# AlgoLab/RecGraph

Measured on AMD Instinct MI355X. Metric: aligned reads/sec (-m 8 recombination, 1 kbp reads, 10k-row/32-path graph), higher is better.
Workload: dtype int16

## Files before the change

### recgraph_amd/csrc/rg_path_driver.hip

```cpp
#include <algorithm>
#include <chrono>
#include <cstdio>
#include <cstdlib>
#include <cstring>

#include "gap/rg_path_gap.hpp"
#include "gap_local/rg_path_gap_local.hpp"
#include "gap_long/rg_path_gap_long.hpp"
#include "gap_xlong/rg_path_gap_xlong.hpp"
#include "gap_xstrands/rg_gap_xstrands.hpp"
#include "edit/rg_path_edit.hpp"
#include "edit_xlong/rg_path_edit_xlong.hpp"
#include "edit_strands/rg_edit_strands.hpp"
#include "rg_kernel_timer.hpp"
#include "rg_path_kernels.hpp"
#include "rg_path_plan.hpp"

namespace rg {

struct PathWorkImpl {
    bool tables = false;
    DevBuf<int> fpoff, fprow, fpslot, rpoff, rprow, rpslot;
    DevBuf<ReadState> state;
    DevBuf<int> roll, mf, wr, mfarg, wrarg, thr, flayer, rlayer;
// ... 433 lines not shown
    RG_TRY(T.run("k_search", [&] { return launch_search(sr, chunk, stream); }));
    RG_TRY(T.inst(launch_need(w.state.p, w.nf.p, w.nr.p, plan.use_rec ? w.nrec.p : nullptr, plan.use_rec ? w.nrrec.p : nullptr, w.need.p, chunk, stream)));
    if (plan.spec) RG_TRY(T.inst(launch_verify(w.state.p, w.lb.p, w.need.p + 4, w.rt_flags.p, chunk, sa.dsel_pick, sa.dsel_pick2, sa.dsel_lo, sa.dsel_hi, stream)));
    return RG_OK;
}

int Run::enqueue_tail() {
    const int C = plan.C;
    LayerArgs la;
    memset(&la, 0, sizeof la);
    la.semi = plan.semi ? 1 : 0;
    la.nwv = plan.nwv;
    la.g = gd; la.sc = sc; la.reads = d_reads; la.read_off = off(); la.state = w.state.p; la.dir_words = plan.dir_words; la.dir_fmt = plan.use16 ? 1 : 0;
    la.layer_stride = plan.layer_stride; la.fpoff = w.fpoff.p; la.fprow = w.fprow.p; la.fpslot = w.fpslot.p;
    la.rpoff = w.rpoff.p; la.rprow = w.rprow.p; la.rpslot = w.rpslot.p;
    la.rev = 0; la.dirs = w.fdirs.p; la.dirs_stride = plan.fdirs_stride; la.layer = w.flayer.p;
    const int win = plan.layer_window;
    auto layer = [&]() {
        if (win) return launch_layer_window(la, chunk, C, win, stream);
        return plan.layer16 ? launch_layer16(la, chunk, C, stream) : launch_layer(la, chunk, C, stream);
    };
    auto fwd_side = [&]() { la.rev = 0; la.dirs = w.fdirs.p; la.dirs_stride = plan.fdirs_stride; la.layer = w.flayer.p; };
    auto rev_side = [&]() { la.rev = 1; la.dirs = w.rdirs.p; la.dirs_stride = plan.rdirs_stride; la.layer = w.rlayer.p; };
    const char* family = win ? LAYER_WINDOW_LOG : "inst:";
    RG_TRY(T.run("k_layer_fwd", layer, family, win != 0));
    if (plan.mode == RG_MODE_RECOMBINATION) {
        rev_side();
        RG_TRY(T.run("k_layer_rev", layer, family, win != 0));
    }
    TraceArgs ta;
    memset(&ta, 0, sizeof ta);
    ta.g = gd; ta.sc = sc; ta.reads = d_reads; ta.read_off = off(); ta.state = w.state.p; ta.rec = d_rec + done;
    ta.ops = d_ops + (long long)done * ops_stride; ta.ops_stride = ops_stride; ta.flayer = w.flayer.p;
    ta.rlayer = w.rlayer.p; ta.layer_stride = plan.layer_stride; ta.fpoff = w.fpoff.p; ta.fprow = w.fprow.p;
    ta.rpoff = w.rpoff.p; ta.rprow = w.rprow.p; ta.nreads = chunk; ta.mode = p.mode; ta.semi = plan.semi ? 1 : 0; ta.nwv = plan.nwv;
    ta.window = win; ta.nfull = w.need.p + NEED_LAYER_FULL;
    RG_TRY(T.run("k_trace", [&] { return launch_trace(ta, C, stream); }));
    if (win) {
        la.only_full = 1;
        fwd_side();
        RG_TRY(T.run("k_layer_full", [&] { return launch_layer16(la, chunk, C, stream); }));
        if (plan.mode == RG_MODE_RECOMBINATION) {
            rev_side();
            RG_TRY(T.run("k_layer_full", [&] { return launch_layer16(la, chunk, C, stream); }));
        }
        ta.window = 0; ta.only_full = 1;
        RG_TRY(T.run("k_trace_full", [&] { return launch_trace(ta, C, stream); }));
    }
    return read_back();
}

int Run::read_back() {
    HIPCHK(hipMemcpyAsync(w.h_sum, d_cells, sizeof(unsigned long long), hipMemcpyDeviceToHost, stream));
    HIPCHK(hipMemcpyAsync(w.h_sum + 5, d_cells + 1, sizeof(unsigned long long), hipMemcpyDeviceToHost, stream));
    HIPCHK(hipMemcpyAsync(w.h_sum + 1, w.need.p, 8 * sizeof(unsigned), hipMemcpyDeviceToHost, stream));
    return T.collect(stats);
}

int Run::enqueue_chunk() {
    HIPCHK(hipMemsetAsync(w.state.p, 0, sizeof(ReadState) * chunk, stream));
    if (plan.gap) return enqueue_pathwise_gap();
    if (plan.edit_strands) return enqueue_pathwise_edit_strands();
    if (plan.edit) return plan.edit_xlong ? enqueue_pathwise_edit_xlong() : enqueue_pathwise_edit();
    SweepArgs sa = sweep_args();
    SeedArgs se;
    se.g = gd; se.state = w.state.p; se.nreads = chunk; se.mode = p.mode; se.sc = sc; se.reads = d_reads; se.read_off = off();
    int rc = plan.mode == RG_MODE_PATHWISE ? enqueue_pathwise(sa, se) : enqueue_recombination(sa, se);
    if (rc) return rc;
    return enqueue_tail();
}

int Run::dump_list_stats() {
    const unsigned* nd = need();
    std::vector<unsigned> hn(chunk), hr(chunk);
    HIPCHK(hipMemcpy(hn.data(), w.nf.p, sizeof(unsigned) * chunk, hipMemcpyDeviceToHost));
    HIPCHK(hipMemcpy(hr.data(), w.nr.p, sizeof(unsigned) * chunk, hipMemcpyDeviceToHost));
    unsigned long long sf = 0, sr = 0;
    for (int i = 0; i < chunk; ++i) { sf += hn[i]; sr += hr[i]; }
    fprintf(stderr, "[rg] chunk %d reads: fwd cand mean %.1f max %u (cap %u), rev cand mean %.1f max %u (cap %u)\n", chunk,
            (double)sf / chunk, nd[0], w.fcap, (double)sr / chunk, nd[1], w.rcap);
    if (plan.use_rec) {
        HIPCHK(hipMemcpy(hn.data(), w.nrec.p, sizeof(unsigned) * chunk, hipMemcpyDeviceToHost));
        HIPCHK(hipMemcpy(hr.data(), w.nrrec.p, sizeof(unsigned) * chunk, hipMemcpyDeviceToHost));
        sf = sr = 0;
        for (int i = 0; i < chunk; ++i) { sf += hn[i]; sr += hr[i]; }
        fprintf(stderr, "[rg] records: forward mean %.1f max %u (cap %u), reverse mean %.1f max %u (cap %u)\n",
                (double)sf / chunk, nd[2], w.frec_cap, (double)sr / chunk, nd[3], w.rrec_cap);
    }
    return RG_OK;
}

int Run::regrow_lists(bool& redo) {
    redo = false;
    if (plan.mode != RG_MODE_RECOMBINATION) return RG_OK;
    const unsigned needf = need()[0], needr = need()[1], needrec = need()[2], needrrec = need()[3];
    if (debug) {
        const int rc = dump_list_stats();
        if (rc) return rc;
    }
    if (plan.use_rec && (needrrec > w.rrec_cap || needrec > w.frec_cap)) {
        const unsigned long long fullrec = (unsigned long long)h.L * WAVE;
        if ((needrrec > w.rrec_cap && w.rrec_cap >= fullrec) || (needrec > w.frec_cap && w.frec_cap >= fullrec))
            return fail(RG_ERR_CAPACITY, "record list overflow at full size");
        while (w.rrec_cap < needrrec) w.rrec_cap = (unsigned)std::min<unsigned long long>(2ull * w.rrec_cap, fullrec);
        while (w.frec_cap < needrec) w.frec_cap = (unsigned)std::min<unsigned long long>(2ull * w.frec_cap, fullrec);
        redo = true;
    }
    if (needf > w.fcap || needr > w.rcap) {
// ... 52 lines not shown
    std::vector<uint8_t> fl((size_t)chunk);
    std::vector<long long> ho((size_t)chunk + 1);
    HIPCHK(hipMemcpy(fl.data(), w.rt_flags.p, (size_t)chunk, hipMemcpyDeviceToHost));
    HIPCHK(hipMemcpy(ho.data(), off(), sizeof(long long) * ((size_t)chunk + 1), hipMemcpyDeviceToHost));
    std::vector<int> idx;
    std::vector<long long> so(1, 0);
    for (int i = 0; i < chunk; ++i)
        if (fl[(size_t)i]) { idx.push_back(i); so.push_back(so.back() + (ho[(size_t)i + 1] - ho[(size_t)i])); }
    const int nr = (int)idx.size();
    int rc;
    if ((rc = w.rt_idx.upload(idx)) || (rc = w.rt_off.upload(so)) || (rc = w.rt_reads.alloc((size_t)so.back() + 1)) ||
        (rc = w.rt_bad.alloc((size_t)nr)) || (rc = w.rt_rec.alloc((size_t)nr)) || (rc = w.rt_ops.alloc((size_t)nr * (size_t)ops_stride)) ||
        (rc = w.rt_cells.alloc(2)))
        return rc;
    HIPCHK(hipMemsetAsync(w.rt_bad.p, 0, (size_t)nr, stream));
    RG_TRY(T.inst(launch_gather_reads(d_reads, off(), w.rt_idx.p, w.rt_off.p, w.rt_reads.p, nr, stream)));
    const PathCtx again{h, gd, p, w.retry, stream, w.rt_cells.p, 0, T, stats, spec_level + 1};
    const PathJob failed{w.rt_reads.p, w.rt_off.p, w.rt_bad.p, nr, max_n, w.rt_rec.p, w.rt_ops.p, ops_stride};
    unsigned long long c2[2] = {0, 0};
    RG_TRY(path_driver_run(again, failed, c2));
    RG_TRY(T.inst(launch_scatter_results(w.rt_idx.p, w.rt_rec.p, w.rt_ops.p, d_rec + done, d_ops + (long long)done * ops_stride, ops_stride, nr, stream)));
    HIPCHK(hipStreamSynchronize(stream));
    cells_perf += c2[1];
    return T.collect(stats);
}

}

int path_driver_vote_table(const HostGraph& h, PathWork& pw, const uint32_t** keys, unsigned* table_mask) {
    if (!pw.impl) pw.impl = new PathWorkImpl();
    const int rc = ensure_tables(h, *pw.impl);
    if (rc) return rc;
    *keys = pw.impl->kmer_keys.p;
    *table_mask = pw.impl->kmer_mask;
    return RG_OK;
}

int path_driver_run(const PathCtx& c, const PathJob& j, unsigned long long* cells ) {
    const HostGraph& h = c.h;
    const rg_params& p = c.p;
    hipStream_t stream = c.stream;
    unsigned long long* d_cells = c.d_cells;
    KernelStats& stats = c.stats;
    const int nreads = j.nreads;
    if (!c.w.impl) c.w.impl = new PathWorkImpl();
    PathWorkImpl& w = *c.w.impl;
    const Options& opt = options();
    PathPlan plan;
    int rc = plan_pathwise(p, PathPlanInput{h.P, h.L, h.fslots, h.rslots, h.max_path_rows, j.max_n}, opt, c.spec_level, plan);
    if (rc || (rc = plan_gap_stage(plan, j.stage))) return rc;
    Run r{h, c.gd, p, w, plan, j.reads, j.off, j.bad, j.max_n, j.rec, j.ops, j.ops_stride, d_cells, stream, stats, c.spec_level, c.T, opt.debug != 0};
    for (int i = 0; i < 36; ++i) r.sc.t[i] = p.scores[i];
    r.h_off = j.h_off;
    if (!w.h_sum) HIPCHK(hipHostMalloc((void**)&w.h_sum, 8 * sizeof(unsigned long long), hipHostMallocDefault));
    if ((rc = w.need.alloc(8)) || (rc = ensure_tables(h, w))) return rc;
    if (w.fcap == 0) { w.fcap = plan.fcap; w.rcap = plan.rcap; w.frec_cap = plan.frec_cap; w.rrec_cap = plan.rrec_cap; }
    size_t budget = (size_t)96 << 30;
    {
        size_t fr = 0, tot = 0;
        if (hipMemGetInfo(&fr, &tot) == hipSuccess) budget = fr / 4 * 3;
        if (c.mem_budget) budget = c.mem_budget;
    }
    unsigned long long cells_done = 0, cells_perf = 0;
    int oom_shift = 0;
    while (r.done < nreads) {
        HIPCHK(hipMemsetAsync(d_cells, 0, 2 * sizeof(unsigned long long), stream));
        HIPCHK(hipMemsetAsync(w.need.p, 0, 8 * sizeof(unsigned), stream));
        const size_t per_read_all = plan.per_read_all(w.fcap, w.rcap, w.frec_cap, w.rrec_cap);
        int maxchunk = (int)std::min<size_t>(8192, std::max<size_t>(1, (budget >> oom_shift) / per_read_all));
        if (opt.chunk_reads > 0) maxchunk = std::min<int>(maxchunk, opt.chunk_reads);
        const double dbg_t0 = r.debug ? now_s() : 0;
        const int chunk = r.chunk = (int)even_chunks(nreads - r.done, maxchunk);
        bool oom = false;
        if ((rc = r.alloc_chunk(&oom))) {
            if (rc == RG_ERR_HIP && oom && chunk > 1 && oom_shift < 12) { ++oom_shift; continue; }
            return rc;
        }
        if (r.debug) fprintf(stderr, "[rg] chunk of %d reads: buffers ready after %.1f ms\n", chunk, (now_s() - dbg_t0) * 1e3);
        if ((rc = r.enqueue_chunk())) return rc;
        if (r.debug) fprintf(stderr, "[rg] chunk of %d reads: done after %.1f ms\n", chunk, (now_s() - dbg_t0) * 1e3);
        if (r.async_err != hipSuccess) return fail(RG_ERR_HIP, std::string("hipMemsetAsync: ") + hipGetErrorString(r.async_err));
        bool redo = false;
        if ((rc = r.regrow_lists(redo))) return rc;
        if (redo) continue;
        const unsigned long long chunk_cells = w.h_sum[0];
        cells_perf += w.h_sum[5];
        const unsigned nretry = r.nretry();
        if (r.debug && (plan.spec || plan.spec4)) fprintf(stderr, "[rg] speculative bound (margin %d): %u of %d reads did not reach it\n", plan.spec_margin, nretry, chunk);
        if (r.debug && plan.spec4 && nretry && (rc = r.dump_spec4_retries())) return rc;
        if (r.debug && plan.dsel && (rc = r.dump_dsel_retries())) return rc;
        if (plan.layer_window) {
            add_stat(stats, "mem:layer_full_reads", (double)r.need()[NEED_LAYER_FULL], 1);
            if (r.debug) fprintf(stderr, "[rg] layer window of %d columns: %u of %d reads took the full-width layers\n", plan.layer_window, r.need()[NEED_LAYER_FULL], chunk);
        }
        if (plan.use_rec) {
            add_stat(stats, "mem:silent_rows", (double)r.need()[NEED_SILENT_ROWS], 1);
            add_stat(stats, "mem:run_rows", (double)r.need()[NEED_RUN_ROWS], 1);
        }
        if (nretry && (rc = r.second_pass(cells_perf))) return rc;
        cells_done += chunk_cells;
        r.done += chunk;
        add_stat(stats, "mem:work_bytes_per_read", (double)per_read_all, 1);
    }
    cells[0] += cells_done;
    cells[1] += cells_perf;
    return RG_OK;
}

}
```

### recgraph_amd/csrc/rg_path_kernels.hpp

```cpp
#pragma once
#include "rg_path_args.hpp"
#include "rg_path_plan.hpp"
#include "rg_launch_log.hpp"
#include "layer_window/rg_layer_window.hpp"

namespace rg {

template <int H>
__device__ __forceinline__ void dir16_decode(unsigned w, unsigned& u16, unsigned& l16) {
    constexpr unsigned LOWH = (1u << H) - 1u;
    const unsigned t = __brev(w);
    u16 = ((t >> 24) & LOWH) | (((t >> 16) & LOWH) << H);
    l16 = ((t >> 8) & LOWH) | ((t & LOWH) << H);
}

struct SweepArgs {
    PathGraphDev g;
    DevScores sc;
    const uint8_t* reads;
    const long long* read_off;
    const uint8_t* bad;
    ReadState* state;
    int* roll;
    int rev;
    int track_best;
    const int* thr;
    const int4* fsteps;
    const int4* rsteps;
    int nfsteps, nrsteps;
    const int4* fsplit;
    const int4* rsplit;
    int use_split;
    const int* lb;
    int brc, maxmatch;
    int semi;
    float rbw;
    int* colmax_out;
    int* colarg_out;
    Cand* cand;
    unsigned cand_cap;
    unsigned* ncand_out;
    uint32_t* dirs;
    long long dirs_stride;
    int dir_words;
    unsigned long long* cells;
    int count_cells;
    int oob;
    int* frec;
    unsigned frec_cap;
    int nwv;
    int gather_ok;
    const unsigned long long* flead;
    const unsigned long long* rlead;
    const unsigned long long* fslead;
    const unsigned long long* rslead;
    int retire;
    int retire_shift;
    const int* order;
    unsigned long long table_members;
    unsigned long long fmembers, rmembers;
    const int* dsel_pick;
    const int* dsel_pick2;
    int dsel_lo, dsel_hi;
    unsigned* runstat;
};
constexpr int NEED_SILENT_ROWS = 6;
constexpr int NEED_RUN_ROWS = 7;

struct ExpandArgs {
    ReadState* state;
    const int* frec;
    unsigned frec_cap;
    const unsigned* nrec;
    Cand* fcand;
    unsigned fcap;
    unsigned* nf;
    const int* wr;
    int wpad;
    int brc;
    const int* knm;
    int rev;
    const long long* read_off;
    float rbw;
    int gcost;
};

struct SeedArgs {
    PathGraphDev g;
    ReadState* state;
    int nreads;
    int mode;
    DevScores sc;
    const uint8_t* reads;
    const long long* read_off;
};

struct ThrArgs {
    const ReadState* state;
    const int* colmax;
    int* thr;
    int wpad;
    int brc;
    int use_bound;
    const int* lb;
};

struct BoundArgs {
    PathGraphDev g;
    ReadState* state;
    const long long* read_off;
    const int* mf; const int* mfarg;
    const int* wr; const int* wrarg;
    int wpad;
    int brc;
    float mrc;
    float rbw;
};

struct Opt0Args {
    PathGraphDev g;
// ... 176 lines not shown
```

### recgraph_amd/csrc/rg_sweep16.hip

```cpp
#include <algorithm>
#include <type_traits>

#include "rg_path_kernels.hpp"
#include "rg_pk16.hpp"

namespace rg {

namespace {

constexpr int NEG32 = INT32_MIN / 4;
typedef unsigned u32x4 __attribute__((ext_vector_type(4)));
typedef unsigned u32x2 __attribute__((ext_vector_type(2)));
__device__ __forceinline__ __amdgpu_buffer_rsrc_t uniform_rsrc(const void* base, unsigned bytes) {
    const unsigned long long u = (unsigned long long)base;
    const unsigned lo = (unsigned)__builtin_amdgcn_readfirstlane((int)(unsigned)u), hi = (unsigned)__builtin_amdgcn_readfirstlane((int)(unsigned)(u >> 32));
    void* p = (void*)(((unsigned long long)hi << 32) | lo);
    return __builtin_amdgcn_make_buffer_rsrc(p, 0, (int)__builtin_amdgcn_readfirstlane((int)bytes), 0x00020000);
}

template <int C>
struct RowOps16 {
    static constexpr int H = C / 2;
    static constexpr unsigned FULL = H >= 16 ? 0xffffffffu : ((((1u << H) - 1u) << 16) | ((1u << H) - 1u));

// ... 145 lines not shown
#define RG_STALL_BEGIN() ((void)0)
#define RG_STALL_END(acc) ((void)0)
#endif

struct PathWords {
    unsigned long long w0, w1, w2, w3;
    __device__ __forceinline__ unsigned long long get(int i) const { return i == 0 ? w0 : (i == 1 ? w1 : (i == 2 ? w2 : w3)); }
    __device__ __forceinline__ void set(int i, unsigned long long v) { if (i == 0) w0 = v; else if (i == 1) w1 = v; else if (i == 2) w2 = v; else w3 = v; }
};

template <int C, int kColmax, bool kRec, bool kWide, bool kSemi>
__global__ __launch_bounds__(64, SWEEP16_WAVES) void k_sweep16(SweepArgs a) {
    static_assert(kColmax == 0 || kColmax == 1, "column maxima with their rows, or none");
    static_assert(!(kColmax == 1 && kRec), "a record sweep tracks no column maxima (k_colmax_rec reads them out of the records): launch_sweep16");
    constexpr int H = C / 2;
    constexpr bool kTrack = kColmax == 1 || kRec;
    constexpr bool kRet = ((kRec && kColmax == 0) || !kTrack) && !kSemi;
    constexpr int NW = kWide ? RG_PW : 1;
    constexpr bool kChain = !kTrack;
    constexpr int KRUN = sweep16_krun(C, !kTrack, kRec && kColmax == 0, kWide);
    static_assert(!(kRec && C <= 16) || KRUN == RG_SWEEP16_RUN_PATHS, "the split step tables (rg_steps.cpp) are built for register runs of RG_SWEEP16_RUN_PATHS paths");
    const int rd = a.order ? a.order[blockIdx.x] : blockIdx.x;
#ifdef RG_SWEEP16_STALLSTAT
    const unsigned long long st_t0 = __builtin_amdgcn_s_memtime();
    unsigned long long st_run = 0, st_nrun = 0, st_gen = 0;
#endif
    const int lane = threadIdx.x;
    const PathGraphDev& g = a.g;
    const int P = g.P;
    const int wpad = C * WAVE;
    const int wrow = H * WAVE;
    ReadState* rs = a.state + rd;
    const long long ro = a.read_off[rd];
    const int n = __builtin_amdgcn_readfirstlane((int)(a.read_off[rd + 1] - ro));
    if (a.bad[rd] || n + 1 > wpad) {
        if (lane == 0 && !a.rev) { rs->status = a.bad[rd] ? ST_BAD_BASE : ST_WOULD_PANIC; }
        return;
    }
    const uint8_t* read = a.reads + ro - 1;
    const bool rev = a.rev;
    const int ncols = rev ? n : n + 1;
    const int GAP = 5;
    extern __shared__ __attribute__((aligned(16))) int lds16[];
    constexpr int EP = kWide ? RG_MAXP : 64;
    constexpr int GTW = C * WAVE > 5 * 64 ? C * WAVE : 5 * 64;
    int* sct = lds16;
    int* endv = lds16 + 64;
    int* endr = endv + EP;
    int* gT = endr + EP;
    int* s2 = gT;
    int* sprof = gT + GTW;
    const int PR_RVL = P, PR_NPROF = P + 1;
    if (lane < 36) sct[lane] = a.sc.t[lane];
    else if (lane < 44) sct[lane] = 0;
    __syncthreads();
    const int gcost = __builtin_amdgcn_readfirstlane(sct[GAP]);
    pair_table(s2, sct, gcost, lane);
    int* rows = a.roll + (long long)rd * (P + 2) * wrow;
    const unsigned lane_row_off = (unsigned)lane * (unsigned)(H * sizeof(int));
    const __amdgpu_buffer_rsrc_t rows_rsrc = uniform_rsrc(rows, (unsigned)((P + 2) * wrow) * 4u);
    auto ld_row = [&](int k, int (&dst)[H]) {
        const int so = k * (int)(wrow * sizeof(int));
        if constexpr (H >= 4) {
#pragma unroll
            for (int r4 = 0; r4 < H / 4; ++r4) {
                const u32x4 v = __builtin_amdgcn_raw_buffer_load_b128(rows_rsrc, (int)lane_row_off + 16 * r4, so, 0);
                dst[4 * r4] = (int)v.x; dst[4 * r4 + 1] = (int)v.y; dst[4 * r4 + 2] = (int)v.z; dst[4 * r4 + 3] = (int)v.w;
            }
        } else {
            const u32x2 v = __builtin_amdgcn_raw_buffer_load_b64(rows_rsrc, (int)lane_row_off, so, 0);
            dst[0] = (int)v.x; dst[1] = (int)v.y;
        }
    };
    auto st_row = [&](int k, const int (&src)[H]) {
        const int so = k * (int)(wrow * sizeof(int));
        if constexpr (H >= 4) {
#pragma unroll
            for (int r4 = 0; r4 < H / 4; ++r4) {
                const u32x4 v = {(unsigned)src[4 * r4], (unsigned)src[4 * r4 + 1], (unsigned)src[4 * r4 + 2], (unsigned)src[4 * r4 + 3]};
                __builtin_amdgcn_raw_buffer_store_b128(v, rows_rsrc, (int)lane_row_off + 16 * r4, so, 0);
                asm volatile("s_nop 1" :: "v"(v));
            }
        } else {
            const u32x2 v = {(unsigned)src[0], (unsigned)src[1]};
            __builtin_amdgcn_raw_buffer_store_b64(v, rows_rsrc, (int)lane_row_off, so, 0);
        }
    };
    unsigned long long pcode[(H + 7) / 8] = {};
    int thrk[(kRec || !kTrack) ? 1 : C];
#define THRK(q) thrk[(kRec || !kTrack) ? 0 : (q)]
    int thz[kRec ? H : 1];
    int minplain2 = 0;
    int thzmin = 0;
    int next_eval = INT32_MAX;
    int minthrk = INT32_MAX;
    int minplain = INT32_MAX;
    const bool tight = a.thr != nullptr || a.oob;
    const int oob = max((int)((float)(n + 1) * (1.0f - a.rbw) / 2.0f), 1);
    auto thr_key = [&](int q, bool member_rule) -> int {
        const int c = lane * C + q;
        const int j = rev ? n - c : c;
        int th = INT32_MAX;
        if (c < ncols && j >= oob && j < n + 1 - oob) {
            if (a.thr) th = a.thr[(long long)rd * wpad + j];
            else if (a.lb) th = a.lb[rd] + a.brc - (n - j) * a.maxmatch;
        }
        if (th == INT32_MAX) return INT32_MAX;
// ... 297 lines not shown
    auto set_keys = [&](int (&bkey)[C], const int (&row)[H], int ks) {
        int k = ks;
        asm volatile("" : "+v"(k));
#pragma unroll
        for (int r = 0; r < H; ++r) {
            bkey[r] = (int)(((unsigned)row[r] << 16) | (unsigned)k);
            bkey[r + H] = (int)(((unsigned)row[r] & 0xffff0000u) | (unsigned)k);
        }
    };
    auto fold_keys = [&](int (&bkey)[C], const int (&row)[H], int ks) {
        int k = ks;
        asm volatile("" : "+v"(k));
#pragma unroll
        for (int r = 0; r < H; ++r) {
            bkey[r] = max(bkey[r], (int)(((unsigned)row[r] << 16) | (unsigned)k));
            bkey[r + H] = max(bkey[r + H], (int)(((unsigned)row[r] & 0xffff0000u) | (unsigned)k));
        }
    };

    auto load_steps = [&](int li_, int (&s)[H]) {
        if (li_ >= 4) [[unlikely]] {
            ld_row(PR_NPROF, s);
            __builtin_amdgcn_s_waitcnt(0x0F70);
            asm volatile("" ::: "memory");
            return;
        }
        const int* sp = sprof + (li_ * WAVE + lane) * H;
        if constexpr (H >= 4) {
#pragma unroll
            for (int r4 = 0; r4 < H / 4; ++r4) {
                const int4 v = reinterpret_cast<const int4*>(sp)[r4];
                s[4 * r4] = v.x; s[4 * r4 + 1] = v.y; s[4 * r4 + 2] = v.z; s[4 * r4 + 3] = v.w;
            }
        } else {
            const int2 v = *reinterpret_cast<const int2*>(sp);
            s[0] = v.x; s[1] = v.y;
        }
    };
    auto keys_ld = [&](int (&key)[C]) {
#pragma unroll
        for (int q = 0; q < C; ++q) key[q] = gT[q * WAVE + lane];
    };
    auto keys_st = [&](const int (&key)[C]) {
#pragma unroll
        for (int q = 0; q < C; ++q) gT[q * WAVE + lane] = key[q];
    };
    int MUw[kWide ? H : 1], MLw[kWide ? H : 1];
    unsigned lmaskw = 0;
    int srcw = 0;
    bool row_open = false;
    constexpr bool kSilent = kRec && kColmax == 0 && !kWide && !kSemi && C <= 16;
    const bool silent_ok = kSilent && (rev || (a.thr == nullptr && a.brc >= 0));
    int* sil = sct + 40;
#ifdef RG_SWEEP16_RETSTAT
    unsigned long long stat_e = 0, stat_n = 0, stat_h = 0;
#endif
    auto retire_eval = [&](int e) {
        PathWords hop{0ull, 0ull, 0ull, 0ull};
        constexpr int EB = !kTrack ? 1 : (C <= 16 ? 4 : 2);
        int rvc[H];
        ld_row(PR_RVL, rvc);
#pragma unroll
        for (int pg = 0; pg < NW; ++pg) {
            unsigned long long todo = needed.get(pg), hp = 0ull;
            while (todo) {
                int kq[EB];
                int tmp[EB][H];
#pragma unroll
                for (int u = 0; u < EB; ++u) {
                    kq[u] = -1;
                    if (todo) {
                        kq[u] = __builtin_ctzll(todo);
                        todo &= todo - 1;
                        ld_row(pg * 64 + kq[u], tmp[u]);
                    }
                }
#pragma unroll
                for (int u = 0; u < EB; ++u) {
                    if (kq[u] < 0) break;
                    int m = pk_add_sat(tmp[u][0], rvc[0]);
#pragma unroll
                    for (int r = 1; r < H; ++r) m = pk_max(m, pk_add_sat(tmp[u][r], rvc[r]));
                    const int v = max(lo16(m), hi16(m));
                    if (__builtin_amdgcn_readlane(dpp_incl_max(v, INT32_MIN), WAVE - 1) < 0) hp |= 1ull << kq[u];
                }
            }
            hop.set(pg, hp);
        }
        if constexpr (kSilent) {
            if (silent_ok) { sil[0] |= (int)(unsigned)hop.w0; sil[1] |= (int)(unsigned)(hop.w0 >> 32); }
        }
        const int nw = kWide ? (P + 63) >> 6 : 1;
        const unsigned long long* lead = (rev ? a.rlead : a.flead) + (long long)e * (64 * nw) * nw;
        PathWords nd{0ull, 0ull, 0ull, 0ull};
#pragma unroll
        for (int pg = 0; pg < NW; ++pg) nd.set(pg, needed.get(pg) & ~hop.get(pg));
#ifdef RG_SWEEP16_RETSTAT
        const unsigned long long nd_first = nd.w0;
#endif
        if constexpr (!kWide) {
            const unsigned long long lead_k = lane < P ? lead[lane] : 0ull;
            for (;;) {
                const unsigned long long ad = __ballot(((needed.w0 >> lane) & 1ull) && !((nd.w0 >> lane) & 1ull) && (lead_k & nd.w0) != 0ull);
                if (!ad) break;
                nd.w0 |= ad;
            }
// ... 2 lines not shown
                bool grown = false;
#pragma unroll
                for (int pg = 0; pg < NW; ++pg) {
                    bool leads = false;
                    if (pg < nw && pg * 64 + lane < P && ((needed.get(pg) >> lane) & 1ull) && !((nd.get(pg) >> lane) & 1ull)) {
#pragma unroll
                        for (int w = 0; w < NW; ++w)
                            if (w < nw) leads = leads || (lead[(long long)(pg * 64 + lane) * nw + w] & nd.get(w)) != 0ull;
                    }
                    const unsigned long long ad = __ballot(leads);
                    if (ad) { nd.set(pg, nd.get(pg) | ad); grown = true; }
                }
                if (!grown) break;
            }
        }
        needed = nd;
#ifdef RG_SWEEP16_RETSTAT
        stat_e += 1ull; stat_n += (unsigned long long)__popcll(nd.w0); stat_h += (unsigned long long)__popcll(nd_first);
#endif
    };
    while (t < nsteps) {
        int w0, w1;
        unsigned long long gmask;
        if (kRet && next_eval != INT32_MAX) {
            if ((t >> 6) != blk) fetch(t, w0, w1, gmask);
            if (t >= next_eval) [[unlikely]] {
                retire_eval(t >> a.retire_shift);
                next_eval = (t | ((1 << a.retire_shift) - 1)) + 1;
                live = block_live();
            }
            const unsigned long long m = live >> (t & (WAVE - 1));
            if (m == 0ull) { t = (t | (WAVE - 1)) + 1; continue; }
            t += __builtin_ctzll(m);
        }
        fetch(t, w0, w1, gmask);
        const int i = w0 & 0xfffff;
        const int li = (w0 >> 20) & 7;
        const int flags = (((w0 >> 23) & 7) == F_INNER && ((w0 >> 26) & 63) != 0) ? 7 : ((w0 >> 23) & 7);
        const int slot = w1 & 0xfffff;
        const int kbase = kWide ? ((w1 >> 29) & 3) * 64 : 0;
        const bool cont = kWide && w1 < 0;
        const int ga = kbase + ((flags & F_INNER) ? __builtin_ctzll(gmask | (1ull << 63)) : ((w0 >> 26) & 63));
        const int nm = __popcll(gmask);
        const int run_left = (flags & F_INNER) ? ((w0 >> 26) & 63) : 0;
        const int page = kWide ? (w1 >> 29) & 3 : 0;
        const unsigned long long gm = kRet ? (gmask & word_of(needed, page)) : gmask;
        const int nme = kRet ? __popcll(gm) : nm;
        if (kRet && gm == 0ull) {
            if (run_left == 0) {
                if (flags & F_FIRST) row_open = false;
                if (track && (flags & F_LAST) && row_open) {
                    int key[C];
                    keys_ld(key);
                    row_end(i, ((w1 >> 20) & 511) - 1, key);
                }
                if (flags & F_LAST) row_open = false;
            }
            ++t;
            continue;
        }
        int went = 1, wide_n = 0, wide_total = nm, wide_needed = 0;
        PathWords wide_gw{0ull, 0ull, 0ull, 0ull};
        int wide_ids[KRUN > 0 ? KRUN : 1];
        bool wide_sel = false;
        if (kWide && (flags & F_INNER) && run_left > 0) {
#pragma unroll
            for (int kk = 0; kk < KRUN; ++kk) wide_ids[kk] = 0;
            auto add = [&](unsigned long long m, int base) {
                while (m) {
                    const int id = base + __builtin_ctzll(m);
                    m &= m - 1;
#pragma unroll
                    for (int kk = 0; kk < KRUN; ++kk) if (kk == wide_n) wide_ids[kk] = id;
                    ++wide_n;
                }
            };
            add(gm, kbase);
            wide_gw.set(page, gm);
            wide_needed = nme;
            wide_sel = (gmask & word_of(dsel_w, page)) != 0ull;
            while (t + went < nsteps) {
                const int nw1 = peek_w1(t + went);
                if (nw1 >= 0) break;
                const unsigned long long mm = peek_gm(t + went);
                const int pg = (nw1 >> 29) & 3;
                wide_total += __popcll(mm);
                add(mm & word_of(needed, pg), pg * 64);
                wide_gw.set(pg, mm & word_of(needed, pg));
                wide_needed += __popcll(mm & word_of(needed, pg));
                wide_sel = wide_sel || (mm & word_of(dsel_w, pg)) != 0ull;
                ++went;
            }
        }
        const bool wide_run = kWide && KRUN > 0 && (flags & F_INNER) && run_left > 0 && wide_n >= 1 && wide_n <= KRUN;
        struct MemberIter {
            PathWords w;
            int pg;
            __device__ __forceinline__ int next() {
                while (pg < NW) {
                    const unsigned long long m = w.get(pg);
                    if (m) { w.set(pg, m & (m - 1)); return pg * 64 + __builtin_ctzll(m); }
                    ++pg;
                }
                return -1;
            }
        };
        const int g_nm = kWide ? wide_total : nm, g_nme = kWide ? wide_needed : nme;
        if ((kRec ? kColmax == 0 : !track) && a.gather_ok && !semi_end && (flags & F_INNER) && g_nm > KRUN &&
            (!kWide || run_left > 0) && (!kRet || g_nme > KRUN) && run_left * (GATHER_PER_MEMBER_ROW * (g_nm - 1) - GATHER_PER_ROW) >= GATHER_PER_MEMBER_RUN * (g_nm - 1)) {
            const int R = (w0 >> 26) & 63;
            const int ka = ga;
            int A[H], G[H];
            __syncthreads();
#pragma unroll
            for (int r = 0; r < H; ++r) A[r] = 0;
            ld_row(ka, A);
#if defined(RG_SWEEP16_STALLSTAT) && RG_SWEEP16_STALLSTAT == 2
            { RG_STALL_BEGIN(); RG_STALL_END(st_run); ++st_nrun; }
#endif
            if (kRec && track) {
                int bd[H], bk[H];
#pragma unroll
                for (int r = 0; r < H; ++r) { bd[r] = 0; bk[r] = pack16(ka, ka); }
                MemberIter it{kWide ? wide_gw : PathWords{gm, 0ull, 0ull, 0ull}, 0};
                it.w.set(ka >> 6, it.w.get(ka >> 6) & ~(1ull << (ka & 63)));
                int nx[H];
                int kn = it.next();
                if (kn >= 0) ld_row(kn, nx);
                while (kn >= 0) {
                    const int k = kn;
                    int cur[H];
#pragma unroll
                    for (int r = 0; r < H; ++r) cur[r] = nx[r];
                    kn = it.next();
                    if (kn >= 0) ld_row(kn, nx);
                    int kk = k;
                    asm volatile("" : "+v"(kk));
                    const int K2 = (int)(((unsigned)kk << 16) | (unsigned)kk);
#pragma unroll
                    for (int r = 0; r < H; ++r) {
                        const int d = pk_sub_sat(cur[r], A[r]);
                        const int lt = pk_sign(pk_sub_sat(d, bd[r]));
                        bd[r] = pk_max(bd[r], d);
                        bk[r] = bfi(lt, bk[r], K2);
                    }
                }
#pragma unroll
                for (int r = 0; r < H; ++r) {
                    gT[r * WAVE + lane] = (int)(((unsigned)bd[r] << 16) | ((unsigned)bk[r] & 0xffffu));
                    gT[(r + H) * WAVE + lane] = (int)(((unsigned)bd[r] & 0xffff0000u) | ((unsigned)bk[r] >> 16));
                }
            }
            {
                int gl = lane;
                asm volatile("" : "+v"(gl));
#pragma unroll
                for (int r = 0; r < H; ++r) { const int w = r * WAVE + gl; G[r] = pack16(2 * w, 2 * w + 1); }
            }
            __syncthreads();
            int ri = i, rli = li, rslot = slot, rw1 = w1;
            for (int step = 0;; ++step) {
                const int g_i = gcost;
                const int g0 = kSemi ? 0 : g_i;
                int s[H], MU[H], ML[H], XU[H], XL[H];
                load_steps(rli, s);
                int lmax_unused;
                RowOps16<C>::alpha(A, s, g_i, g0, lane, XU, XL, lmax_unused);
                const bool gdirs = kWide ? ((kColmax == 0 || dirs != nullptr) && (wide_sel || edge_row(ri))) : want_dirs(gmask, 0, ri);
                if (gdirs) store_dirs(rslot, XU, XL);
                const unsigned lmask = RowOps16<C>::masks(XU, XL, MU, ML);
                const int src = RowOps16<C>::src_lane(lmask, lane);
                RowOps16<C>::template member<true>(G, MU, lane, MU, ML, lmask, src);
                cells += (unsigned long long)g_nm;
                done += 2ull;
                if (kRec && track) {
                    int bv[H], K2[H];
                    constexpr int HS = 31 - __builtin_clz(H * WAVE);
// ... 114 lines not shown
            };
            constexpr bool kRowsInBody = !kChain && !kWide;
            if constexpr (!kRowsInBody) ld_run(rnm);
#if defined(RG_SWEEP16_STALLSTAT) && RG_SWEEP16_STALLSTAT == 3
            const unsigned long long st_rb = __builtin_amdgcn_s_memtime();
#endif
            int ri = i, rli = li, rslot = slot, rw1 = w1, rfl = 7;
            int rleft = run_left;
            bool tail = false;
            for (;;) {
            tail = false; rfl = 7;
            auto run_rows = [&](auto rn_tag, auto lean_tag) __attribute__((always_inline)) {
            constexpr int RN = decltype(rn_tag)::value;
            constexpr bool kLean = decltype(lean_tag)::value;
            const unsigned long long run_sel = kWide ? (wide_sel ? ~0ull : 0ull) : rgm;
            const int run_page = 0;
            if constexpr (kRowsInBody) ld_run(RN);
            unsigned nrows = 0;
            while (true) {
                int cnt = 1;
                if constexpr (!kWide) {
                    if (!tail) cnt = max(min(min(rleft, WAVE - (t & (WAVE - 1))), nsteps - t), 1);
                }
                nrows += (unsigned)cnt;
                int idx = t & (WAVE - 1);
                for (int left = cnt;;) {
                const int g_i = gcost;
                const int g0 = kSemi ? 0 : g_i;
                int XU[H], XL[H];
#if defined(RG_SWEEP16_STALLSTAT) && RG_SWEEP16_STALLSTAT == 3
                ++st_nrun;
#endif
                int s[H];
                load_steps(rli, s);
                int lmax;
                RowOps16<C>::alpha(rr[0], s, g_i, g0, lane, XU, XL, lmax);
                if constexpr (!kLean) {
                    if (kWide ? ((kColmax == 0 || dirs != nullptr) && (wide_sel || edge_row(ri))) : want_dirs(run_sel, run_page, ri)) store_dirs(rslot, XU, XL);
                }
                if constexpr (RN > 1) {
                    int MU[H], ML[H];
                    const unsigned lmask = RowOps16<C>::masks(XU, XL, MU, ML);
                    const int src = RowOps16<C>::src_lane(lmask, lane);
                    int SEL[H];
                    RowOps16<C>::select_steps(SEL, s, MU, g_i, g0, lane);
                    int zl[KRUN > 0 ? KRUN : 1], vlo[KRUN > 0 ? KRUN : 1];
#pragma unroll
                    for (int kk = 1; kk < KRUN; ++kk)
                        if (kk < RN) { RowOps16<C>::member_p1(rr[kk], SEL, MU, ML, lmask, zl[kk], vlo[kk]); zl[kk] = __shfl(zl[kk], src, WAVE); }
#pragma unroll
                    for (int kk = 1; kk < KRUN; ++kk)
                        if (kk < RN) RowOps16<C>::member_p2(rr[kk], ML, lmask, zl[kk], vlo[kk]);
                }
                if (kRec && kColmax == 0 && tail) {
                    if (track) {
                        if (rfl & F_FIRST) row_open = false;
                        int key[C];
                        if (row_open) { keys_ld(key); fold_keys(key, rr[0], mk[0]); } else set_keys(key, rr[0], mk[0]);
#pragma unroll
                        for (int kk = 1; kk < KRUN; ++kk) if (kk < RN) fold_keys(key, rr[kk], mk[kk]);
                        row_open = true;
                        int tri = ri, tw1 = rw1;
                        if constexpr (kLean) asm volatile("" : "+s"(tri), "+s"(tw1));
                        if (rfl & F_LAST) { row_end(tri, ((tw1 >> 20) & 511) - 1, key); row_open = false; }
                        else keys_st(key);
                    }
                } else if constexpr (kLean) {
                } else if (track && kRec && kColmax == 0) {
                    int bv[H];
#pragma unroll
                    for (int r = 0; r < H; ++r) bv[r] = rr[0][r];
#pragma unroll
                    for (int kk = 1; kk < KRUN; ++kk)
                        if (kk < RN) {
#pragma unroll
                            for (int r = 0; r < H; ++r) bv[r] = pk_max(bv[r], rr[kk][r]);
                        }
                    const int knm_row = ((rw1 >> 20) & 511) - 1;
                    int acc = -1;
                    bool fine = true;
                    if constexpr (RN == 1 && kRec) {
                        if (knm_row >= 0) fine = __any(((unsigned)pk_sub_sat(lmax, thzmin) & 0x80008000u) != 0x80008000u);
                    }
                    if (!fine) {
                    } else if (knm_row >= 0) [[likely]] {
#pragma unroll
                        for (int r = 0; r < H; ++r) acc &= pk_sub_sat(bv[r], thz[kRec ? r : 0]);
                    } else {
                        int m = bv[0];
#pragma unroll
                        for (int r = 1; r < H; ++r) m = pk_max(m, bv[r]);
                        acc = pk_sub_sat(m, minplain2);
                    }
                    const bool lhit = ((unsigned)acc & 0x80008000u) != 0x80008000u;
                    if (__any(lhit)) {
                        bool mine;
                        int4* rp = rec_slot(ri, lhit, mine);
#pragma unroll
                        for (int half = 0; half < 2; ++half) {
                            int hk[H];
#pragma unroll
                            for (int kk = 0; kk < KRUN; ++kk)
                                if (kk < RN) {
                                    int kv = mk[kk];
                                    asm volatile("" : "+v"(kv));
#pragma unroll
                                    for (int r = 0; r < H; ++r) {
                                        const int key = half == 0 ? (int)(((unsigned)rr[kk][r] << 16) | (unsigned)kv)
                                                                  : (int)(((unsigned)rr[kk][r] & 0xffff0000u) | (unsigned)kv);
                                        hk[r] = kk == 0 ? key : max(hk[r], key);
                                    }
                                }
                            rec_half(rp, mine, half, hk);
                        }
                    }
                } else if (track) {
                    int key[C];
                    set_keys(key, rr[0], mk[0]);
// ... 124 lines not shown
        } else {
        const int g_i = gcost;
        const int g0 = kSemi ? 0 : g_i;
        int s[H];
        load_steps(li, s);
        int MUl[kWide ? 1 : H], MLl[kWide ? 1 : H];
        unsigned lmaskl = 0;
        int srcl = 0;
        int (&MU)[H] = *reinterpret_cast<int (*)[H]>(kWide ? MUw : MUl);
        int (&ML)[H] = *reinterpret_cast<int (*)[H]>(kWide ? MLw : MLl);
        unsigned& lmask = kWide ? lmaskw : lmaskl;
        int& src = kWide ? srcw : srcl;
        {
            unsigned long long rest = cont ? gm : gm & ~(1ull << (ga - kbase));
            cells += (unsigned long long)nm;
            done += (unsigned long long)nme;
            int nxt[H];
            int knext = -1;
            if (rest) {
                knext = kbase + __builtin_ctzll(rest);
                rest &= rest - 1;
                ld_row(knext, nxt);
            }
            int key[C];
            bool have = false;
            if (track) {
                if (flags & F_FIRST) row_open = false;
                have = row_open;
                if (have) keys_ld(key);
            }
            if (!cont) {
                int rowa[H];
                ld_row(ga, rowa);
#if defined(RG_SWEEP16_STALLSTAT) && RG_SWEEP16_STALLSTAT == 1
                { RG_STALL_BEGIN(); RG_STALL_END(st_gen); }
#endif
                int XU[H], XL[H];
                int lmax_unused;
                RowOps16<C>::alpha(rowa, s, g_i, g0, lane, XU, XL, lmax_unused);
                st_row(ga, rowa);
                bool wd = want_dirs(gmask, page, i);
                if (kWide && !wd && t + 1 < nsteps) wd = peek_w1(t + 1) < 0;
                if (wd) store_dirs(slot, XU, XL);
                lmask = RowOps16<C>::masks(XU, XL, MU, ML);
                src = RowOps16<C>::src_lane(lmask, lane);
                if (track) {
                    if (!have) set_keys(key, rowa, ga); else fold_keys(key, rowa, ga);
                    have = true;
                }
                if (semi_end) end_fold(ga, i, rowa);
            }
            int SEL[H];
            RowOps16<C>::select_steps(SEL, s, MU, g_i, g0, lane);
            while (knext >= 0) {
                const int k = knext;
                int cur[H];
#pragma unroll
                for (int r = 0; r < H; ++r) cur[r] = nxt[r];
                if (rest) {
                    knext = kbase + __builtin_ctzll(rest);
                    rest &= rest - 1;
                    ld_row(knext, nxt);
                } else knext = -1;
                RowOps16<C>::member(cur, SEL, lane, MU, ML, lmask, src);
                st_row(k, cur);
                if (track) fold_keys(key, cur, k);
                if (semi_end) end_fold(k, i, cur);
            }
            if (track) {
                row_open = true;
                if (e_flags & F_LAST) row_end(e_i, ((e_w1 >> 20) & 511) - 1, key);
                else keys_st(key);
            }
        }
        }
        if (semi_end && (e_flags & F_LAST)) end_row_done(e_i);
        if (e_flags & F_LAST) row_open = false;
        if (e_adv) ++t;
    }

    if (kColmax == 1 && a.colmax_out) {
#pragma unroll
        for (int q = 0; q < C; ++q) {
            const int c = lane * C + q;
            if (c < ncols) {
                a.colmax_out[(long long)rd * wpad + (rev ? n - c : c)] = ckey[kColmax == 1 ? q : 0] == INT32_MIN ? NEG32 : (ckey[kColmax == 1 ? q : 0] >> 16) + c * gcost;
                if (a.colarg_out) a.colarg_out[(long long)rd * wpad + (rev ? n - c : c)] = (crow[kColmax == 1 ? q : 0] << 8) | (ckey[kColmax == 1 ? q : 0] & 255);
            }
        }
    }
    if (a.ncand_out && lane == 0) a.ncand_out[rd] = ncand;
    __syncthreads();
    if (!rev && !kSemi) {
        const int ql = n % C, ln = n / C;
        for (int k = lane; k < P; k += WAVE) {
            const int pv = rows[(long long)k * wrow + ln * H + (ql % H)];
            rs->sink_val[k] = (kRet && !((word_of(needed, k >> 6) >> (k & 63)) & 1ull)) ? NEG32 : (ql >= H ? hi16(pv) : lo16(pv)) + n * gcost;
        }
    }
    if (semi_end) {
        for (int k = lane; k < P; k += WAVE) { rs->sink_val[k] = endv[k]; rs->path_end_row[k] = endr[k]; }
        if (lane == ln_end) { rs->s0 = gbest_val; rs->end_row_best = gbest_row; rs->seed_path = gbest_path; }
    }
    if constexpr (kSilent) {
        if (lane == 0 && a.runstat) { atomicAdd(a.runstat, (unsigned)sil[2]); atomicAdd(a.runstat + 1, (unsigned)sil[3]); }
    }
    if (lane == 0 && a.count_cells) {
        const unsigned long long all = kRet && a.table_members ? a.table_members : cells;
#ifdef RG_SWEEP16_STALLSTAT
        {
            const unsigned long long tot = __builtin_amdgcn_s_memtime() - st_t0;
            atomicAdd(a.cells, (tot >> 8) | ((st_gen >> 8) << 32));
            atomicAdd(a.cells + 1, (st_run >> 8) | (st_nrun << 32));
            return;
        }
#endif
#ifdef RG_SWEEP16_RETSTAT
        if (kRet) { atomicAdd(a.cells, stat_e | (stat_n << 32)); atomicAdd(a.cells + 1, stat_h | ((unsigned long long)(rev ? 0 : 1) << 48)); return; }
#endif
        atomicAdd(a.cells, all * (unsigned long long)(n + 1));
        atomicAdd(a.cells + 1, done * (unsigned long long)(n + 1));
    }
}

template <int C>
__global__ __launch_bounds__(256) void k_expand(ExpandArgs a) {
    const int rd = blockIdx.x;
    const int lane = threadIdx.x & (WAVE - 1), wv = threadIdx.x / WAVE, nwv = blockDim.x / WAVE;
    ReadState* rs = a.state + rd;
    if (rs->status & (ST_BAD_BASE | ST_WOULD_PANIC)) return;
    const unsigned nrec = a.nrec[rd];
    if (nrec > a.frec_cap) { if (threadIdx.x == 0) rs->status |= ST_OVERFLOW; return; }
    const int bound = rs->bound;
    const int nread = (int)(a.read_off[rd + 1] - a.read_off[rd]);
    const int oob = max((int)((float)(nread + 1) * (1.0f - a.rbw) / 2.0f), 1);
    const int* base = a.frec + (long long)rd * a.frec_cap * (4 + C);
    Cand* out = a.fcand + (long long)rd * a.fcap;
    const int* wr = a.wr + (long long)rd * a.wpad;
    constexpr int LPR = C / 4, RPW = WAVE / LPR;
    const int part = lane % LPR, sub = lane / LPR;
    for (unsigned t0 = wv * RPW; t0 < nrec; t0 += nwv * RPW) {
        const unsigned t = t0 + sub;
        if (t >= nrec) continue;
        const int* rp = base + (long long)t * (4 + C);
        const int rl = rp[0];
        const int4 k4 = *reinterpret_cast<const int4*>(rp + 4 + 4 * part);
        const int keys[4] = {k4.x, k4.y, k4.z, k4.w};
        const int knm = a.knm[rl >> 6];
#pragma unroll
        for (int e = 0; e < 4; ++e) {
            const int cc = (rl & 63) * C + 4 * part + e;
            if (cc >= (a.rev ? nread : nread + 1)) continue;
            const int key = keys[e] + cc * a.gcost * 65536;
            const int val = key >> 16;
            const int col = a.rev ? nread - cc : cc;
            if (col < oob || col >= nread + 1 - oob) continue;
            if (val + wr[col] - a.brc < bound) continue;
            if (knm >= 0 && key <= knm) continue;
// ... 301 lines not shown
```

Baseline: 151,200.

## Skip key folds for silent paths in recombination sweep and add fold stats

```diff
diff --git a/recgraph_amd/csrc/rg_path_driver.hip b/recgraph_amd/csrc/rg_path_driver.hip
--- a/recgraph_amd/csrc/rg_path_driver.hip
+++ b/recgraph_amd/csrc/rg_path_driver.hip
@@ -509,8 +509,8 @@
 
 int Run::read_back() {
     HIPCHK(hipMemcpyAsync(w.h_sum, d_cells, sizeof(unsigned long long), hipMemcpyDeviceToHost, stream));
-    HIPCHK(hipMemcpyAsync(w.h_sum + 5, d_cells + 1, sizeof(unsigned long long), hipMemcpyDeviceToHost, stream));
-    HIPCHK(hipMemcpyAsync(w.h_sum + 1, w.need.p, 8 * sizeof(unsigned), hipMemcpyDeviceToHost, stream));
+    HIPCHK(hipMemcpyAsync(w.h_sum + 1 + NEED_WORDS / 2, d_cells + 1, sizeof(unsigned long long), hipMemcpyDeviceToHost, stream));
+    HIPCHK(hipMemcpyAsync(w.h_sum + 1, w.need.p, NEED_WORDS * sizeof(unsigned), hipMemcpyDeviceToHost, stream));
     return T.collect(stats);
 }
 
@@ -669,8 +669,8 @@
     Run r{h, c.gd, p, w, plan, j.reads, j.off, j.bad, j.max_n, j.rec, j.ops, j.ops_stride, d_cells, stream, stats, c.spec_level, c.T, opt.debug != 0};
     for (int i = 0; i < 36; ++i) r.sc.t[i] = p.scores[i];
     r.h_off = j.h_off;
-    if (!w.h_sum) HIPCHK(hipHostMalloc((void**)&w.h_sum, 8 * sizeof(unsigned long long), hipHostMallocDefault));
-    if ((rc = w.need.alloc(8)) || (rc = ensure_tables(h, w))) return rc;
+    if (!w.h_sum) HIPCHK(hipHostMalloc((void**)&w.h_sum, (2 + NEED_WORDS / 2) * sizeof(unsigned long long), hipHostMallocDefault));
+    if ((rc = w.need.alloc(NEED_WORDS)) || (rc = ensure_tables(h, w))) return rc;
     if (w.fcap == 0) { w.fcap = plan.fcap; w.rcap = plan.rcap; w.frec_cap = plan.frec_cap; w.rrec_cap = plan.rrec_cap; }
     size_t budget = (size_t)96 << 30;
     {
@@ -682,7 +682,7 @@
     int oom_shift = 0;
     while (r.done < nreads) {
         HIPCHK(hipMemsetAsync(d_cells, 0, 2 * sizeof(unsigned long long), stream));
-        HIPCHK(hipMemsetAsync(w.need.p, 0, 8 * sizeof(unsigned), stream));
+        HIPCHK(hipMemsetAsync(w.need.p, 0, NEED_WORDS * sizeof(unsigned), stream));
         const size_t per_read_all = plan.per_read_all(w.fcap, w.rcap, w.frec_cap, w.rrec_cap);
         int maxchunk = (int)std::min<size_t>(8192, std::max<size_t>(1, (budget >> oom_shift) / per_read_all));
         if (opt.chunk_reads > 0) maxchunk = std::min<int>(maxchunk, opt.chunk_reads);
@@ -701,7 +701,7 @@
         if ((rc = r.regrow_lists(redo))) return rc;
         if (redo) continue;
         const unsigned long long chunk_cells = w.h_sum[0];
-        cells_perf += w.h_sum[5];
+        cells_perf += w.h_sum[1 + NEED_WORDS / 2];
         const unsigned nretry = r.nretry();
         if (r.debug && (plan.spec || plan.spec4)) fprintf(stderr, "[rg] speculative bound (margin %d): %u of %d reads did not reach it\n", plan.spec_margin, nretry, chunk);
         if (r.debug && plan.spec4 && nretry && (rc = r.dump_spec4_retries())) return rc;
@@ -713,6 +713,14 @@
         if (plan.use_rec) {
             add_stat(stats, "mem:silent_rows", (double)r.need()[NEED_SILENT_ROWS], 1);
             add_stat(stats, "mem:run_rows", (double)r.need()[NEED_RUN_ROWS], 1);
+            add_stat(stats, "mem:key_folds", (double)r.need()[NEED_KEY_FOLDS], 1);
+            add_stat(stats, "mem:key_rows", (double)r.need()[NEED_KEY_ROWS], 1);
+            add_stat(stats, "mem:key_rows_hit", (double)r.need()[NEED_KEY_ROWS_HIT], 1);
+            const unsigned* kn = r.need();
+            add_stat(stats, "mem:key_folds_saved", (double)kn[NEED_KEY_SAVED_GATHER] + (double)kn[NEED_KEY_SAVED_GENERAL] + (double)kn[NEED_KEY_SAVED_TAIL], 1);
+            add_stat(stats, "mem:key_saved_gather", (double)kn[NEED_KEY_SAVED_GATHER], 1);
+            add_stat(stats, "mem:key_saved_general", (double)kn[NEED_KEY_SAVED_GENERAL], 1);
+            add_stat(stats, "mem:key_saved_tail", (double)kn[NEED_KEY_SAVED_TAIL], 1);
         }
         if (nretry && (rc = r.second_pass(cells_perf))) return rc;
         cells_done += chunk_cells;
diff --git a/recgraph_amd/csrc/rg_path_kernels.hpp b/recgraph_amd/csrc/rg_path_kernels.hpp
--- a/recgraph_amd/csrc/rg_path_kernels.hpp
+++ b/recgraph_amd/csrc/rg_path_kernels.hpp
@@ -66,6 +66,13 @@
 };
 constexpr int NEED_SILENT_ROWS = 6;
 constexpr int NEED_RUN_ROWS = 7;
+constexpr int NEED_KEY_FOLDS = 8;
+constexpr int NEED_KEY_ROWS = 9;
+constexpr int NEED_KEY_ROWS_HIT = 10;
+constexpr int NEED_KEY_SAVED_GATHER = 11;
+constexpr int NEED_KEY_SAVED_GENERAL = 12;
+constexpr int NEED_KEY_SAVED_TAIL = 13;
+constexpr int NEED_WORDS = 14;
 
 struct ExpandArgs {
     ReadState* state;
diff --git a/recgraph_amd/csrc/rg_sweep16.hip b/recgraph_amd/csrc/rg_sweep16.hip
--- a/recgraph_amd/csrc/rg_sweep16.hip
+++ b/recgraph_amd/csrc/rg_sweep16.hip
@@ -221,7 +221,7 @@
     int* sprof = gT + GTW;
     const int PR_RVL = P, PR_NPROF = P + 1;
     if (lane < 36) sct[lane] = a.sc.t[lane];
-    else if (lane < 44) sct[lane] = 0;
+    else if (lane < 50) sct[lane] = 0;
     __syncthreads();
     const int gcost = __builtin_amdgcn_readfirstlane(sct[GAP]);
     pair_table(s2, sct, gcost, lane);
@@ -625,6 +625,18 @@
     constexpr bool kSilent = kRec && kColmax == 0 && !kWide && !kSemi && C <= 16;
     const bool silent_ok = kSilent && (rev || (a.thr == nullptr && a.brc >= 0));
     int* sil = sct + 40;
+    enum { KS_GATHER = 7, KS_GENERAL = 8, KS_TAIL = 9 };
+    auto silent_set = [&]() -> unsigned long long {
+        return ((unsigned long long)(unsigned)__builtin_amdgcn_readfirstlane(sil[1]) << 32) | (unsigned)__builtin_amdgcn_readfirstlane(sil[0]);
+    };
+    auto key_stat = [&](int folds, bool closed, unsigned before, int saved, int place) {
+        if constexpr (kSilent) {
+            if (folds) sil[4] += folds;
+            if (closed) sil[5] += 1;
+            if (closed && ncand != before) sil[6] += 1;
+            if (saved) sil[place] += saved;
+        }
+    };
 #ifdef RG_SWEEP16_RETSTAT
     unsigned long long stat_e = 0, stat_n = 0, stat_h = 0;
 #endif
@@ -733,7 +745,9 @@
                 if (track && (flags & F_LAST) && row_open) {
                     int key[C];
                     keys_ld(key);
+                    const unsigned before = ncand;
                     row_end(i, ((w1 >> 20) & 511) - 1, key);
+                    key_stat(0, true, before, 0, KS_GENERAL);
                 }
                 if (flags & F_LAST) row_open = false;
             }
@@ -803,7 +817,12 @@
                 int bd[H], bk[H];
 #pragma unroll
                 for (int r = 0; r < H; ++r) { bd[r] = 0; bk[r] = pack16(ka, ka); }
-                MemberIter it{kWide ? wide_gw : PathWords{gm, 0ull, 0ull, 0ull}, 0};
+                unsigned long long pm = gm;
+                if constexpr (kSilent) {
+                    pm = gm & ~silent_set();
+                    key_stat(0, false, 0u, __popcll(gm & ~pm & ~(1ull << ka)), KS_GATHER);
+                }
+                MemberIter it{kWide ? wide_gw : PathWords{pm, 0ull, 0ull, 0ull}, 0};
                 it.w.set(ka >> 6, it.w.get(ka >> 6) & ~(1ull << (ka & 63)));
                 int nx[H];
                 int kn = it.next();
@@ -1024,9 +1043,13 @@
                     for (int kk = 1; kk < KRUN; ++kk)
                         if (kk < RN) RowOps16<C>::member_p2(rr[kk], ML, lmask, zl[kk], vlo[kk]);
                 }
-                if (kRec && kColmax == 0 && tail) {
+                bool tail_eager = kRec && kColmax == 0 && tail;
+                if (tail_eager && (rfl & F_FIRST)) row_open = false;
+                if constexpr (kSilent && kLean) {
+                    if (tail_eager && row_open && !(rfl & F_LAST)) { tail_eager = false; key_stat(0, false, 0u, RN, KS_TAIL); }
+                }
+                if (tail_eager) {
                     if (track) {
-                        if (rfl & F_FIRST) row_open = false;
                         int key[C];
                         if (row_open) { keys_ld(key); fold_keys(key, rr[0], mk[0]); } else set_keys(key, rr[0], mk[0]);
 #pragma unroll
@@ -1034,8 +1057,10 @@
                         row_open = true;
                         int tri = ri, tw1 = rw1;
                         if constexpr (kLean) asm volatile("" : "+s"(tri), "+s"(tw1));
+                        const unsigned before = ncand;
                         if (rfl & F_LAST) { row_end(tri, ((tw1 >> 20) & 511) - 1, key); row_open = false; }
                         else keys_st(key);
+                        key_stat(RN, (rfl & F_LAST) != 0, before, 0, KS_GENERAL);
                     }
                 } else if constexpr (kLean) {
                 } else if (track && kRec && kColmax == 0) {
@@ -1266,6 +1291,9 @@
             }
             int SEL[H];
             RowOps16<C>::select_steps(SEL, s, MU, g_i, g0, lane);
+            unsigned long long mute = 0ull;
+            int nfold = cont ? 0 : 1, nmute = 0;
+            if constexpr (kSilent) { if (silent_ok && next_eval != INT32_MAX) mute = silent_set(); }
             while (knext >= 0) {
                 const int k = knext;
                 int cur[H];
@@ -1278,13 +1306,18 @@
                 } else knext = -1;
                 RowOps16<C>::member(cur, SEL, lane, MU, ML, lmask, src);
                 st_row(k, cur);
-                if (track) fold_keys(key, cur, k);
+                if (track) {
+                    if (kSilent && ((mute >> (k & 63)) & 1ull)) ++nmute;
+                    else { fold_keys(key, cur, k); ++nfold; }
+                }
                 if (semi_end) end_fold(k, i, cur);
             }
             if (track) {
                 row_open = true;
+                const unsigned before = ncand;
                 if (e_flags & F_LAST) row_end(e_i, ((e_w1 >> 20) & 511) - 1, key);
                 else keys_st(key);
+                key_stat(nfold, (e_flags & F_LAST) != 0, before, nmute, KS_GENERAL);
             }
         }
         }
@@ -1317,7 +1350,10 @@
         if (lane == ln_end) { rs->s0 = gbest_val; rs->end_row_best = gbest_row; rs->seed_path = gbest_path; }
     }
     if constexpr (kSilent) {
-        if (lane == 0 && a.runstat) { atomicAdd(a.runstat, (unsigned)sil[2]); atomicAdd(a.runstat + 1, (unsigned)sil[3]); }
+        if (lane == 0 && a.runstat) {
+#pragma unroll
+            for (int w = 0; w < 8; ++w) atomicAdd(a.runstat + w, (unsigned)sil[2 + w]);
+        }
     }
     if (lane == 0 && a.count_cells) {
         const unsigned long long all = kRet && a.table_members ? a.table_members : cells;
```

After: 154,200, median of 6. 2.0% higher.
